# cvangysel/SERT

Hardware: AMD Instinct MI355X
Metric: training_pairs_per_sec (higher is better)
Workload: dtype f32; 1 GPU; C2 LSE: VectorSpaceLanguageModel (NCE z=10, Adam) V_w=100000 V_e=1000 d=128 window=10 batch=65536; global_batch=65536, per_gpu_batch=65536, parallelism=dp1, id_dtype=uint32, seed=0, instance_weights=1, dataset_instances=4194304, dataset_batches=64

## Files before the change

### include/sert_hip_debug.h

```cpp
#ifndef SERT_HIP_DEBUG_H
#define SERT_HIP_DEBUG_H

#include "sert_hip.h"

#ifdef __cplusplus
extern "C" {
#endif

int sert_debug_update_counts(sert_model* m, int64_t* out, int n);

int sert_debug_poison_scratch(sert_model* m);

int sert_debug_row_lists(const uint32_t* allbits, int world, int rank, int64_t num_batches, int64_t bit_words,
                         int64_t rows_per_rank, int64_t vocab, int64_t batch, int32_t* serve_cnt,
                         int32_t* fetch_cnt, int32_t* serve_rows, int32_t* fetch_rows, int32_t* union_rows,
                         int32_t* ptr, int32_t* ent, int64_t capacity, int64_t* sizes);

int sert_debug_word_index_sum(const void* ids, int id_bytes, int64_t num_batches, int B, int n, int vocab, int row_groups,
                              int dense_heavy, int64_t batch, const float* src, int d, float divisor, float* grad_out,
                              int64_t* stats);

int sert_debug_ll_rank_distributions(int device, const float* P, const int64_t* offsets, int64_t num_queries, int32_t V,
                                     int32_t k, int32_t* idx_out, float* score_out, float* joint_entropy_out,
                                     float* token_entropy_out, int32_t* status_out);

int sert_bench_gemm(int device, int ta, int tb, int epi, int M, int N, int K, int splits,
                    int iters, double* avg_us);

int sert_debug_gemm(int device, int ta, int tb, int epi, int M, int N, int K, const float* A, const float* B,
                    const float* bias, float* C);

int sert_debug_gemm_splitk(int device, int M, int N, int K, int splits, const float* A, const float* B, float* out);

int sert_debug_gemm_longk(int device, int tb, int M, int N, int K, int splits, const float* A, const float* B, float* C);

enum { SERT_MEMBENCH_COPY = 0, SERT_MEMBENCH_READ = 1, SERT_MEMBENCH_GATHER = 2, SERT_MEMBENCH_OPTIMIZER = 3 };
int sert_bench_memory(int device, int kind, size_t bytes, size_t table_bytes, int row_bytes,
                      int window, size_t gap_bytes, int blocks, int iters, double* avg_us);

struct sert_reval;
int sert_debug_reval_chunks(struct sert_reval* r);

// ... 5 lines not shown
```

### sert_amd/_capi.py

```python
import ctypes
import os

import numpy as np

_HERE = os.path.dirname(os.path.abspath(__file__))
LIB_PATH = os.environ.get('SERT_LIB') or os.path.join(_HERE, 'libsert_hip.so')

KIND_LOGLINEAR, KIND_VECTORSPACE, KIND_VECTORSPACE_SOFTMAX = 0, 1, 2
SPLIT_TRAIN, SPLIT_VALIDATE = 0, 1
LL_STATUS_DEVICE, LL_STATUS_HOST = 0, 1
REVAL_NDCG, REVAL_MAP, REVAL_RECIP_RANK, REVAL_P5, REVAL_NUM_REL_RET, REVAL_NUM_METRICS = 0, 1, 2, 3, 4, 5

T_RW, T_RE, T_W, T_B = 0, 1, 2, 3
T_STATE0_RW, T_STATE0_RE, T_STATE0_W, T_STATE0_B = 4, 5, 6, 7
T_STATE1_RW, T_STATE1_RE, T_STATE1_W, T_STATE1_B = 8, 9, 10, 11
T_GRAD_RW, T_GRAD_RE, T_GRAD_W, T_GRAD_B = 12, 13, 14, 15
T_ACT_H, T_ACT_T, T_ACT_DA, T_ACT_DH, T_ACT_ROWLOSS = 16, 17, 18, 19, 20

COMM_ID_BYTES = 128

EXPORTS = [
    'sert_create', 'sert_destroy', 'sert_last_error', 'sert_device_info', 'sert_device_count',
    'sert_set_tensor', 'sert_get_tensor', 'sert_tensor_size', 'sert_set_step', 'sert_get_step',
    'sert_set_eval_draws', 'sert_get_eval_draws', 'sert_negatives_of_step',
    'sert_upload_dataset', 'sert_train_batch', 'sert_hint_next_batch', 'sert_train_batches',
    'sert_eval_batch', 'sert_eval_batches',
    'sert_predict_project', 'sert_predict_tokens', 'sert_ll_rank_queries', 'sert_score_topk',
    'sert_reval_create', 'sert_reval_run', 'sert_reval_destroy',
    'sert_scorer_create', 'sert_scorer_destroy', 'sert_scorer_topk', 'sert_scorer_scores',
    'sert_host_alloc', 'sert_host_free',
    'sert_comm_unique_id', 'sert_comm_init', 'sert_comm_init_host', 'sert_comm_destroy', 'sert_comm_stats',
    'sert_synchronize', 'sert_timing_enable', 'sert_timing_reset', 'sert_timing_count',
    'sert_timing_name', 'sert_timing_avg_us', 'sert_timing_launches', 'sert_bench_gemm', 'sert_debug_gemm', 'sert_debug_gemm_splitk', 'sert_debug_gemm_longk', 'sert_bench_memory', 'sert_debug_row_lists', 'sert_debug_word_index_sum',
    'sert_debug_update_counts', 'sert_debug_poison_scratch', 'sert_debug_ll_rank_distributions', 'sert_debug_reval_chunks',
    'sert_profile_range_push', 'sert_profile_range_pop',
]


_F32P, _I64P = ctypes.POINTER(ctypes.c_float), ctypes.POINTER(ctypes.c_int64)
ALLTOALL_FN = ctypes.CFUNCTYPE(ctypes.c_int, ctypes.c_void_p, _F32P, _I64P, _I64P, _F32P, _I64P, _I64P)


class SertConfig(ctypes.Structure):
    _fields_ = [
        ('struct_size', ctypes.c_uint32),
        ('kind', ctypes.c_int32),
        ('batch_size', ctypes.c_int32),
        ('global_batch_size', ctypes.c_int32),
        ('window_size', ctypes.c_int32),
        ('vocab_size', ctypes.c_int32),
        ('num_entities', ctypes.c_int32),
        ('word_dim', ctypes.c_int32),
        ('entity_dim', ctypes.c_int32),
        ('num_negatives', ctypes.c_int32),
        ('id_bytes', ctypes.c_int32),
        ('device', ctypes.c_int32),
        ('keep_grads', ctypes.c_int32),
        ('deterministic', ctypes.c_int32),
        ('inference_only', ctypes.c_int32),
        ('lambda_', ctypes.c_float),
        ('lr', ctypes.c_float),
        ('beta1', ctypes.c_float),
        ('beta2', ctypes.c_float),
        ('eps', ctypes.c_float),
        ('seed', ctypes.c_uint64),
    ]

# ... 268 lines not shown
    def comm_stats(self):
        v = (ctypes.c_double * 8)()
        check(self._lib.sert_comm_stats(self._h, v, 8))
        return {'world': int(v[0]), 'exchange': {0: 'none', 1: 'zero1', 2: 'rows'}[int(v[1])],
                'bytes_per_step': float(v[2]), 'zero1_bytes_per_step': float(v[3]),
                'transport': {0: 'none', 1: 'rccl', 2: 'host'}[int(v[4])], 'steps': int(v[5]),
                'rows_fetched_per_batch': float(v[6]), 'rows_served_per_batch': float(v[7])}

    def synchronize(self):
        check(self._lib.sert_synchronize(self._h))

    def timing_enable(self, on=True):
        check(self._lib.sert_timing_enable(self._h, int(on)))

    def timing_launches(self):
        n = self._lib.sert_timing_count(self._h)
        return {self._lib.sert_timing_name(self._h, i).decode():
                self._lib.sert_timing_launches(self._h, i) for i in range(n)}

    def timing_reset(self):
        check(self._lib.sert_timing_reset(self._h))

    def poison_scratch(self):
        self._lib.sert_debug_poison_scratch.argtypes = [ctypes.c_void_p]
        check(self._lib.sert_debug_poison_scratch(self._h))

    def update_counts(self):
        v = (ctypes.c_int64 * 10)()
        self._lib.sert_debug_update_counts.argtypes = [ctypes.c_void_p, ctypes.POINTER(ctypes.c_int64), ctypes.c_int]
        check(self._lib.sert_debug_update_counts(self._h, v, 10))
        names = ('dense', 'lazy', 'skip_32_1', 'skip_64_1', 'skip_32_3', 'skip_64_2', 'skip_64_3', 'skip_64_4', 'skip_full', 'skip_sparse')
        return dict(zip(names, (int(x) for x in v)))

    def timings(self):
        n = self._lib.sert_timing_count(self._h)
        return {self._lib.sert_timing_name(self._h, i).decode():
                self._lib.sert_timing_avg_us(self._h, i) for i in range(n)}


def comm_unique_id():
    buf = ctypes.create_string_buffer(COMM_ID_BYTES)
    check(load().sert_comm_unique_id(buf))
    return buf.raw


def _concat_queries(token_lists):
    lengths = np.fromiter((len(t) for t in token_lists), dtype=np.int64, count=len(token_lists))
    offsets = np.zeros(len(token_lists) + 1, dtype=np.int64)
    np.cumsum(lengths, out=offsets[1:])
    tokens = np.ascontiguousarray(np.concatenate([np.asarray(t, dtype=np.int64) for t in token_lists])
                                  if len(token_lists) else np.zeros(0, np.int64), dtype=np.int32)
    return tokens, offsets


def _ll_rank_call(num_entities, offsets, k, call, num_tokens):
    q = offsets.size - 1
    kk = num_entities if k is None or k >= num_entities else int(k)
    idx = np.empty((q, kk), dtype=np.int32)
    score = np.empty((q, kk), dtype=np.float32)
    joint_h = np.empty(q, dtype=np.float32)
    token_h = np.empty(num_tokens, dtype=np.float32)
    status = np.empty(q, dtype=np.int32)
    outs = [a.ctypes.data for a in (idx, score, joint_h, token_h, status)]
    check(call(-1 if k is None else int(k), outs))
    return idx, score, joint_h, token_h, status, offsets

# ... 299 lines not shown
```

### sert_amd/csrc/host/api_data_train.inc

```

int sert_upload_dataset(sert_model* m, int split, const void* x, const int32_t* y_int,
                        const int64_t* csr_indptr, const int32_t* csr_indices,
                        const float* csr_data, const float* w, int64_t N) {
    if (!m) SERT_FAIL("null model");
    invalidate_speculation(m);
    m->hint_next = -1;
    if (split != SERT_SPLIT_TRAIN && split != SERT_SPLIT_VALIDATE) SERT_FAIL("bad split");
    if (N < 0) SERT_FAIL("negative instance count");
    if (N > 0 && !x) SERT_FAIL("x is null");
    if (N > 0 && !y_int && !(csr_indptr && csr_indices && csr_data)) SERT_FAIL("no labels given");
    if (is_vs(m) && N > 0 && !y_int) SERT_FAIL("vectorspace requires int labels (models.py:933-934)");
    SERT_HIP(hipSetDevice(m->cfg.device));
    if (N > 0) {
        const size_t toks = (size_t)N * m->cfg.window_size;
        const uint32_t Vw = (uint32_t)m->cfg.vocab_size;
        bool ok = true;
        SERT_ID_DISPATCH(m->cfg.id_bytes, {
            const IdT* xi = (const IdT*)x;
            uint32_t mx = 0;
            for (size_t i = 0; i < toks; ++i) mx = std::max<uint32_t>(mx, (uint32_t)xi[i]);
            ok = mx < Vw;
        });
        if (!ok) SERT_FAIL("token id >= vocab_size in x");
        const int32_t Ve = m->cfg.num_entities;
// ... 128 lines not shown
                d.dense_cnt_of.resize((size_t)nb);
                for (int64_t b = 0; b < nb; ++b) d.dense_cnt_of[(size_t)b] = wi.batches[(size_t)b].dense_cnt;
            }
            SERT_TRY(dmalloc(&d.idx_dense_words, hw.size()));
            SERT_HIP(hipMemcpyAsync(d.idx_dense_words, hw.data(), hw.size() * sizeof(int32_t), hipMemcpyHostToDevice, s));
            SERT_HIP(hipStreamSynchronize(s));
            if (!m->hpart)
                SERT_TRY(dmalloc(&m->hpart, (size_t)std::max(cdiv(B, heavy_rows_fused(B)), cdiv(B, kHeavyRowsPerBlock)) * kHeavyMax *
                                               (size_t)(is_vs(m) ? m->cfg.word_dim : m->cfg.num_entities)));
        } else {
            for (auto& bxx : wi.batches) bxx.dense_cnt = 0;
        }
        d.idx_batches = wi.batches;
        if ((size_t)wi.max_part_rows + 1 > m->wpart_rows) {
            (void)hipFree(m->wpart);
            m->wpart_rows = (size_t)wi.max_part_rows + 1;
            SERT_TRY(dmalloc(&m->wpart, m->wpart_rows * m->cfg.word_dim));
        }
    }
    SERT_HIP(hipStreamSynchronize(s));
    return 0;
}

int sert_train_batch(sert_model* m, int64_t batch_index, const int64_t* negatives, float* loss_out) {
    refresh_gemm_choice();
    if (!m) SERT_FAIL("null model");
    SERT_HIP(hipSetDevice(m->cfg.device));
    static const bool no_spin = variant_knob("SERT_NO_SPIN") != nullptr;
    const int64_t hint = m->hint_next;
    m->hint_next = -1;
    m->lazy_next = hint;
    auto prefetch_next = [&]() -> int {
        const DataSplit& ds = m->split[SERT_SPLIT_TRAIN];
        if (hint < 0 || m->timing.enabled || m->cfg.keep_grads) return 0;
        if ((hint + 1) * (int64_t)m->cfg.batch_size > ds.N) return 0;
        if (can_speculate_step(m)) {
            bool fused = false;
            SERT_TRY(step_forward_backward(m, ds, hint, nullptr, &fused));
            m->spec_fb_batch = hint;
            m->spec_fb_step = m->step;
        } else if (is_vs(m) && !is_fs(m)) {
            if (m->xr_on) SERT_TRY(xr_fetch_params(m, hint));
            SERT_TRY(vs_project(m, ds, hint));
            m->projected_batch = hint;
        } else if (m->xr_on) {
            SERT_TRY(xr_fetch_params(m, hint));
        }
        return 0;
    };
    if (m->timing.enabled || no_spin) {
        SERT_TRY(train_step_async(m, batch_index, negatives, m->d_loss));
        SERT_HIP(hipMemcpyAsync(m->h_loss, m->d_loss, 3 * sizeof(float), hipMemcpyDeviceToHost, m->stream));
        SERT_HIP(hipEventRecord(m->ev_loss, m->stream));
        SERT_TRY(prefetch_next());
        SERT_HIP(hipEventSynchronize(m->ev_loss));
        timing_collect(m);
        if (loss_out) *loss_out = m->h_loss[0];
        return 0;
    }
    SERT_TRY(train_step_async(m, batch_index, negatives, m->h_loss_dev, true));
    SERT_TRY(prefetch_next());
    const unsigned want = m->loss_seq;
    volatile unsigned* flag = reinterpret_cast<volatile unsigned*>(m->h_loss + 4);
    {
        const auto t_spin0 = std::chrono::steady_clock::now();
        double next_query_ms = 50.0;
        for (unsigned spins = 1; *flag != want; ++spins) {
            if ((spins & 0xfff) != 0) continue;
            const double waited_ms = std::chrono::duration<double, std::milli>(std::chrono::steady_clock::now() - t_spin0).count();
            if (waited_ms < next_query_ms) continue;
            next_query_ms = waited_ms + 50.0;
            const hipError_t q = hipStreamQuery(m->stream);
            if (q == hipSuccess) {
                if (*flag == want) break;
                SERT_FAIL("training step completed without publishing its loss");
            }
            if (q != hipErrorNotReady) SERT_HIP(q);
        }
    }
    __atomic_thread_fence(__ATOMIC_ACQUIRE);
    if (loss_out) *loss_out = m->h_loss[0];
    return 0;
}

int sert_hint_next_batch(sert_model* m, int64_t next_batch_index) {
    if (!m) SERT_FAIL("null model");
    m->hint_next = next_batch_index;
    return 0;
}

int sert_train_batches(sert_model* m, const int64_t* batch_indices, int64_t count, float* losses_out) {
    refresh_gemm_choice();
    if (!m || !batch_indices || count < 0) SERT_FAIL("bad argument");
    m->hint_next = -1;
// ... 191 lines not shown
```

### sert_amd/csrc/host/api_debug.inc

```

int sert_debug_poison_scratch(sert_model* m) {
    if (!m) SERT_FAIL("null argument");
    if (m->spec_fb_batch >= 0) SERT_FAIL("a run-ahead step is in flight (sert_hint_next_batch): its gradients live in the scratch");
    SERT_HIP(hipSetDevice(m->cfg.device));
    SERT_HIP(hipDeviceSynchronize());
    if (!m->gflat) return 0;
    std::vector<uint32_t> h(m->gflat_alloc, 0x7fc00000u);
    if (m->run_start) {
        const size_t V4 = round_up((size_t)m->cfg.num_entities, 4);
        for (size_t i = 0; i < V4; ++i) { h[m->gflat_count + i] = 0u; h[m->gflat_count + V4 + i] = 1u; }
    }
    SERT_HIP(hipMemcpy(m->gflat, h.data(), h.size() * sizeof(uint32_t), hipMemcpyHostToDevice));
    return 0;
}

int sert_debug_update_counts(sert_model* m, int64_t* out, int n) {
    if (!m || !out || n < 1 || n > 10) SERT_FAIL("bad argument");
    for (int i = 0; i < n; ++i) out[i] = m->upd_counts[i];
    return 0;
}

int sert_debug_row_lists(const uint32_t* allbits, int world, int rank, int64_t num_batches, int64_t bit_words,
                         int64_t rows_per_rank, int64_t vocab, int64_t batch, int32_t* serve_cnt, int32_t* fetch_cnt,
                         int32_t* serve_rows, int32_t* fetch_rows, int32_t* union_rows, int32_t* ptr, int32_t* ent,
                         int64_t capacity, int64_t* sizes) {
    if (!allbits || world < 1 || rank < 0 || rank >= world || batch < 0 || batch >= num_batches || !sizes)
        SERT_FAIL("bad argument");
    RowExchangeLists L;
    build_row_exchange(allbits, world, rank, num_batches, bit_words, rows_per_rank, vocab, L);
    const RowExchangeBatch& xb = L.batches[(size_t)batch];
    sizes[0] = xb.serve_total; sizes[1] = xb.fetch_total; sizes[2] = xb.nunion; sizes[3] = xb.nent; sizes[4] = L.max_xfer_rows;
    if (std::max<int64_t>(std::max(xb.serve_total, xb.fetch_total), std::max(xb.nunion + 1, xb.nent)) > capacity)
        SERT_FAIL("capacity too small");
    for (int q = 0; q < world; ++q) { serve_cnt[q] = xb.serve_cnt[(size_t)q]; fetch_cnt[q] = xb.fetch_cnt[(size_t)q]; }
    std::copy_n(L.serve_rows.begin() + xb.serve_off, xb.serve_total, serve_rows);
    std::copy_n(L.fetch_rows.begin() + xb.fetch_off, xb.fetch_total, fetch_rows);
    std::copy_n(L.union_rows.begin() + xb.union_off, xb.nunion, union_rows);
    std::copy_n(L.ptr.begin() + xb.ptr_off, xb.nunion + 1, ptr);
    std::copy_n(L.ent.begin() + xb.ent_off, xb.nent, ent);
    return 0;
}

int sert_debug_word_index_sum(const void* ids, int id_bytes, int64_t num_batches, int B, int n, int vocab, int row_groups,
                              int dense_heavy, int64_t batch, const float* src, int d, float divisor, float* grad_out,
                              int64_t* stats) {
    if (!ids || !src || !grad_out || !stats || num_batches <= 0 || B <= 0 || n <= 0 || vocab <= 0 || d <= 0 || batch < 0 ||
        batch >= num_batches || (id_bytes != 1 && id_bytes != 2 && id_bytes != 4))
        SERT_FAIL("bad argument");
    WordIndex wi;
    bool ok = true;
    SERT_ID_DISPATCH(id_bytes, ok = build_word_index<IdT>((const IdT*)ids, num_batches, B, n, vocab, false, wi,
// ... 353 lines not shown
```

### sert_amd/csrc/host/optimizer_and_loss.inc

```

static int reduce_rowloss(sert_model* m, hipStream_t st) {
    const int B = m->cfg.batch_size;
    int nb = std::min(kOptBlocks, cdiv(B, 256));
    m->loss_from_rows = false;
    if (is_vs(m) && !is_fs(m) && m->nce_loss_partials > 0) nb = m->nce_loss_partials;
    else if (!is_dp(m) && B <= 8192) {
        m->loss_from_rows = true;
        nb = B;
    } else hipLaunchKernelGGL(sum_partial, dim3(nb), dim3(256), 0, st, m->rowloss, (size_t)B, m->red_loss);
    if (is_dp(m))
        hipLaunchKernelGGL(partials_to_scalar, dim3(1), dim3(256), 0, st, m->red_loss, nb, m->g_loss);
    m->n_loss_partials = nb;
    return 0;
}

static void launch_stream_opt(sert_model* m, hipStream_t st, float* p, float* g, float* s0, float* s1, size_t count,
                              int nb, const AdamArgs& aa, const AdadeltaArgs& da, float* sq,
                              const uint32_t* bits, unsigned row_len, float* sq_new = nullptr) {
    const bool keep = m->cfg.keep_grads != 0;
    const int rows_mode = kRowsAll;
    if (is_vs(m)) {
        if (keep) hipLaunchKernelGGL((adam_l2<true>), dim3(nb), dim3(256), 0, st, p, g, s0, s1, count, aa, sq, bits, row_len, rows_mode, sq_new);
        else      hipLaunchKernelGGL((adam_l2<false>), dim3(nb), dim3(256), 0, st, p, g, s0, s1, count, aa, sq, bits, row_len, rows_mode, sq_new);
    } else {
// ... 261 lines not shown
        launch_stream_opt(m, ss, t.p, t.g, t.s0, t.s1, t.n, re_nb, aa, da, m->red_sq + re_sq_lo, nullptr, 1u,
                          m->re_sq + re_nxt * re_cap);
        m->re_sq_for[re_nxt] = m->step + 1;
        SERT_HIP(hipEventRecord(m->ev_re, ss));
        m->re_pending = true;
    }
    {
        ScopedTimer t(m, TG_FINALIZE);
        const float inv_batch = 1.0f / (float)c.global_batch_size;
        const float reg_scale = c.lambda_ > 0.f ? c.lambda_ / (2.0f * (float)c.global_batch_size) : 0.f;
        const float* lp = is_dp(m) ? m->g_loss : (m->loss_from_rows ? m->rowloss : m->red_loss);
        const int nl = is_dp(m) ? 1 : n_loss_partials;
        unsigned* flag = publish ? reinterpret_cast<unsigned*>(loss_dst + 4) : nullptr;
        if (tail_splits > 0) {
            if (m->dw_side_first) SERT_HIP(hipStreamWaitEvent(m->stream, m->ev_dense, 0));
            TailArgs ta;
            ta.part = m->part; ta.splits = tail_splits; ta.stride = m->tail_stride;
            ta.W = m->W; ta.b = m->b; ta.s0_w = m->s0_w; ta.s1_w = m->s1_w; ta.s0_b = m->s0_b; ta.s1_b = m->s1_b;
            ta.g_w = m->g_w; ta.g_b = m->g_b;
            ta.n_w = (unsigned)m->n_w; ta.n_b = (unsigned)m->n_b;
            ta.aa = aa;
            ta.loss_partials = lp; ta.n_loss = nl;
            ta.sq_partials = m->red_sq; ta.n_sq = n_sq;
            const bool alt = defer_re || (defer_small && re_nb > 0);
            ta.sq_alt = alt ? m->re_sq + re_cur * re_cap : nullptr;
            ta.sq_alt_lo = alt ? re_sq_lo : 0;
            ta.sq_alt_hi = alt ? re_sq_lo + re_nb : 0;
            ta.inv_batch = inv_batch; ta.reg_scale = reg_scale;
            ta.out = loss_dst; ta.host_flag = flag; ta.seq = publish ? ++m->loss_seq : 0u;
            ta.blk = m->tail_blk;
            if (++m->tail_launch_seq == 0) ++m->tail_launch_seq;
            ta.launch_seq = m->tail_launch_seq;
            const int nb = cdiv((int64_t)(m->n_w + m->n_b), 64);
            if (c.keep_grads) hipLaunchKernelGGL((vs_tail<true>), dim3(nb), dim3(1024), 0, m->stream, ta);
            else              hipLaunchKernelGGL((vs_tail<false>), dim3(nb), dim3(1024), 0, m->stream, ta);
        } else
        hipLaunchKernelGGL(finalize_loss, dim3(1), dim3(256), 0, m->stream, lp, nl, m->red_sq,
                           n_sq, inv_batch, reg_scale, loss_dst, flag, publish ? ++m->loss_seq : 0u,
                           is_dp(m) ? (const float*)m->g_sq : (const float*)nullptr);
    }
    if (any_ag) {
        SERT_HIP(hipEventRecord(m->ev_ag_done, m->comm_stream));
        SERT_HIP(hipStreamWaitEvent(m->stream, m->ev_ag_done, 0));
    }
    return 0;
}

static size_t zero_from(const sert_model* m) {
    static const bool all = variant_knob("SERT_ZERO_GRE") != nullptr;
    if (!all && m->cfg.kind == SERT_KIND_VECTORSPACE && !m->epart && m->n_re > 0 && m->g_re == m->gflat + m->ar_split)
        return m->ar_split + round_up(m->pt_pad[1], 4);
    return m->ar_split;
}

static bool egrad_writes_every_row(const sert_model* m) { return m->epart != nullptr || zero_from(m) > m->ar_split; }

static bool fused_prologue_applies_with(const sert_model* m, bool touched) {
    return is_vs(m) && !is_fs(m) && !m->timing.enabled && m->nstreams >= 2 && touched &&
           m->cfg.num_negatives > 0 && (m->gflat_alloc - zero_from(m)) % 4 == 0;
}
static bool fused_prologue_applies(const sert_model* m) { return fused_prologue_applies_with(m, m->use_touched); }
static void launch_fused_prologue(sert_model* m) {
    const int64_t count = (int64_t)m->cfg.batch_size * m->cfg.num_negatives;
    hipLaunchKernelGGL(vs_sample_negatives, dim3(grid_for((count + 3) / 4)), dim3(256), 0, m->stream, m->neg,
                       count, (int64_t)m->rank * count, (uint32_t)m->cfg.num_entities, m->cfg.seed,
                       (uint64_t)m->step * 2, reinterpret_cast<float4*>(m->gflat + zero_from(m)),
                       (m->gflat_alloc - zero_from(m)) / 4, (uint4*)nullptr, (size_t)0);
}
// ... 49 lines not shown
            SERT_HIP(hipMemsetAsync(m->gflat, 0, m->gflat_alloc * sizeof(float), pre));
        }
        if (!(is_vs(m) && !is_fs(m) && pre != m->stream)) SERT_TRY(owned_sum_of_squares(m, pre));
    }
    if (is_fs(m)) {
        SERT_TRY(fs_forward<true>(m, ds, batch_index));
        SERT_TRY(fs_backward(m, ds, batch_index));
        SERT_TRY(reduce_rowloss(m, m->stream));
    } else if (is_vs(m)) {
        if (!fused_pre) SERT_TRY(vs_negatives(m, negatives, (uint64_t)m->step * 2, pre));
        if (pre != m->stream) {
            SERT_HIP(hipEventRecord(m->ev_neg, pre));
            SERT_HIP(hipStreamWaitEvent(m->stream, m->ev_neg, 0));
            if (!have_neg && !fused_pre) SERT_TRY(owned_sum_of_squares(m, pre));
        }
        SERT_TRY(vs_loss<true>(m, ds, batch_index));
        SERT_TRY(vs_backward(m, ds, batch_index));
    } else {
        SERT_TRY(ll_forward<true>(m, ds, batch_index));
        SERT_TRY(ll_backward(m, ds, batch_index));
        SERT_TRY(reduce_rowloss(m, m->stream));
    }
    return 0;
}

static bool can_speculate_step(const sert_model* m) {
    if (m->timing.enabled || m->cfg.keep_grads) return false;
    if (is_dp(m)) {
        static const bool dp_off = variant_knob("SERT_DP_RUN_AHEAD") && atoi(variant_knob("SERT_DP_RUN_AHEAD")) == 0;
        return !dp_off && is_vs(m) && !is_fs(m);
    }
    if (is_vs(m) && !is_fs(m)) return use_touched_now(m) && fused_prologue_applies_with(m, true);
    return true;
}

static int train_step_async(sert_model* m, int64_t batch_index, const int64_t* negatives,
                            float* loss_dst, bool publish = false) {
    const DataSplit& ds = m->split[SERT_SPLIT_TRAIN];
    const int B = m->cfg.batch_size;
    if (m->cfg.inference_only) SERT_FAIL("model was created inference_only");
    if (m->comm_dead) SERT_FAIL("the communicator of this data-parallel model was destroyed");
    if (ds.N == 0) SERT_FAIL("no training data uploaded");
    if (batch_index < 0 || (batch_index + 1) * (int64_t)B > ds.N) SERT_FAIL("batch_index out of range");
    if (m->instep.on) ++m->instep.steps;
    const bool have_fb = negatives == nullptr && m->spec_fb_batch == batch_index && m->spec_fb_step == m->step &&
                         can_speculate_step(m);
    bool fused_pre = true;
    if (have_fb) m->spec_fb_batch = -1;
    else discard_run_ahead(m);
    const uint32_t* bits = ds.idx_touched_bits ? ds.idx_touched_bits + (size_t)batch_index * ds.bit_words : nullptr;
    if (!have_fb) SERT_TRY(step_forward_backward(m, ds, batch_index, negatives, &fused_pre));
    SERT_TRY(allreduce_rest(m));
    m->cur_touched_frac = (size_t)batch_index < ds.idx_batches.size()
                              ? (float)ds.idx_batches[(size_t)batch_index].num_distinct / (float)m->cfg.vocab_size : 1.f;
    const uint32_t* next_bits = nullptr;
    if (ds.idx_touched_bits && m->lazy_next >= 0 && (m->lazy_next + 1) * (int64_t)B <= ds.N)
        next_bits = ds.idx_touched_bits + (size_t)m->lazy_next * ds.bit_words;
    SERT_TRY(optimizer_and_loss(m, loss_dst, publish, bits, next_bits));
    if (is_dp(m)) m->comm_steps += 1;
    SERT_HIP(hipGetLastError());
    if (fused_pre) m->step_done_pending = true;
    else { SERT_HIP(hipEventRecord(m->ev_step_done, m->stream)); m->step_done_pending = false; }
    return 0;
}
```

### sert_amd/csrc/host/step_vectorspace.inc

```

static int reduce_rowloss(sert_model* m, hipStream_t st);

static int vs_negatives(sert_model* m, const int64_t* negatives, uint64_t stream_pos, hipStream_t st) {
    const auto& c = m->cfg;
    const int64_t count = (int64_t)c.batch_size * c.num_negatives;
    if (count == 0) return 0;
    if (negatives) {
        const int64_t Ve = c.num_entities;
        for (int64_t i = 0; i < count; ++i)
            if (negatives[i] < 0 || negatives[i] >= Ve) SERT_FAIL("negative sample out of range [0, num_entities)");
        SERT_HIP(hipMemcpyAsync(m->neg_stage, negatives, count * sizeof(int64_t),
                                hipMemcpyHostToDevice, st));
        hipLaunchKernelGGL(convert_i64_to_i32, dim3(grid_for(count)), dim3(256), 0, st,
                           m->neg_stage, m->neg, count);
    } else {
        const int64_t global_offset = (int64_t)m->rank * count;
        hipLaunchKernelGGL(vs_sample_negatives, dim3(grid_for((count + 3) / 4)), dim3(256), 0,
                           st, m->neg, count, global_offset, (uint32_t)c.num_entities,
                           c.seed, stream_pos);
    }
    return 0;
}

static int vs_project(sert_model* m, const DataSplit& ds, int64_t batch_index) {
    const auto& c = m->cfg;
    const int B = c.batch_size, n = c.window_size, dw = c.word_dim, de = c.entity_dim;
    const size_t row0 = (size_t)batch_index * B;
#ifdef SERT_VARIANTS
    if (m->proj_fused && gemm_x3_enabled() && vs_project_fused_ok(B, n, dw, de, m->n_rw)) {
        if (m->T_alt) std::swap(m->T, m->T_alt);
        ScopedTimer t(m, TG_GATHER);
        SERT_ID_DISPATCH(c.id_bytes, {
            const IdT* X = (const IdT*)ds.x + row0 * n;
            hipLaunchKernelGGL((vs_project_x3<IdT>), dim3(vs_project_grid(B, m->num_cus)), dim3(PJ_THREADS), 0, m->stream, X, (const float*)m->rw,
                               (const float*)m->W, (const float*)m->b, m->H, m->T, B, n, dw, de);
        });
        return 0;
    }
#endif
    {
        ScopedTimer t(m, TG_GATHER);
        SERT_ID_DISPATCH(c.id_bytes, {
            const IdT* X = (const IdT*)ds.x + row0 * n;
#ifdef SERT_VARIANTS
            const int nhot = (ds.idx_tok_slot && (size_t)batch_index < ds.dense_cnt_of.size()) ? ds.dense_cnt_of[(size_t)batch_index] : 0;
            if (dw % 4 == 0 && nhot > 0 && (size_t)nhot * dw * sizeof(float) <= 48 * 1024)
                hipLaunchKernelGGL((vs_gather_mean_hot<IdT>), dim3(std::min<int64_t>(grid_for((int64_t)B * dw / 4, 256, 1 << 20), 8 * m->num_cus)),
                                   dim3(256), (size_t)nhot * dw * sizeof(float), m->stream, X, (const uint8_t*)ds.idx_tok_slot + row0 * n,
                                   (const int32_t*)ds.idx_dense_words + (size_t)batch_index * kHeavyMax, nhot, (const float*)m->rw, m->H, B, n, dw);
            else
#endif
            if (dw % 4 == 0)
                hipLaunchKernelGGL((vs_gather_mean<IdT, 4>), dim3(grid_for((int64_t)B * dw / 4, 256, 1 << 20)),
                                   dim3(256), 0, m->stream, X, m->rw, m->H, B, n, dw);
            else
                hipLaunchKernelGGL((vs_gather_mean<IdT, 1>), dim3(grid_for((int64_t)B * dw, 256, 1 << 20)),
                                   dim3(256), 0, m->stream, X, m->rw, m->H, B, n, dw);
        });
    }
    if (m->T_alt) std::swap(m->T, m->T_alt);
    {
        ScopedTimer t(m, TG_GEMM_FWD);
#ifdef SERT_VARIANTS
        if (gemm_strip_ok(B, de, dw, dw, de, false, m->H, m->W))
            launch_gemm_strip<false, EPI_BIAS_TANH>(m->stream, m->H, m->W, m->T, m->b, B, de, dw, dw, de, de);
        else
#endif
            launch_gemm<false, false, EPI_BIAS_TANH>(m->stream, m->H, m->W, m->T, m->b, B, de, dw, dw,
                                                     de, de);
    }
    return 0;
}

static bool ext_events() {
    static const bool on = !(variant_knob("SERT_EXT_EVENTS") && atoi(variant_knob("SERT_EXT_EVENTS")) == 0);
    return on;
}

static bool side_heavy_mode(const sert_model* m);

static bool fork_late_mode(const sert_model* m) {
    static const bool on = !(variant_knob("SERT_FORK_LATE") && atoi(variant_knob("SERT_FORK_LATE")) == 0);
    return on && !side_heavy_mode(m) && ext_events() && !is_dp(m) && !m->timing.enabled && m->nstreams == 2 &&
           m->n_re <= ((size_t)1 << 22) && m->cfg.kind == SERT_KIND_VECTORSPACE;
}

static bool fork_at_nce(const sert_model* m) {
    static const bool on = variant_knob("SERT_FORK_AT") && !strncmp(variant_knob("SERT_FORK_AT"), "nce", 3);
    return on && fork_late_mode(m);
}
// ... 407 lines not shown
```

### sert_amd/csrc/kernels_opt.h

```cpp
#pragma once
#include "common.h"

namespace sert {

#ifndef SERT_OPT_BLOCKS
#define SERT_OPT_BLOCKS 2048
#endif
constexpr int kOptBlocks = SERT_OPT_BLOCKS;

struct AdamArgs {
    float l2k;
    float a_t;
    float b1, b2, eps;
};

__device__ __forceinline__ float sq_acc(float acc, float x) { return __builtin_fmaf(x, x, acc); }

__device__ __forceinline__ void adam_elem(float& p, float& g, float& m, float& v, const AdamArgs& a,
                                          float omb1, float omb2, float& ss, float& ss_new) {
#pragma clang fp contract(off)
    const float pv = p;
    const float l2 = a.l2k * pv;
    const float gv = g + l2;
    ss = sq_acc(ss, pv);
// ... 595 lines not shown
        b += __shfl_xor(b, off);
    }
    if ((threadIdx.x & 63) == 0) { red[0][threadIdx.x >> 6] = a; red[1][threadIdx.x >> 6] = b; }
    __syncthreads();
    const double loss_sum = (red[0][0] + red[0][1]) + (red[0][2] + red[0][3]);
    const double sq_sum = (red[1][0] + red[1][1]) + (red[1][2] + red[1][3]);
    if (threadIdx.x == 0) {
        const float data = (float)loss_sum * inv_batch;
        const float reg = reg_scale * (float)(sq_sum + (extra_sq ? (double)extra_sq[0] : 0.0));
        out[0] = data + reg;
        out[1] = data;
        out[2] = reg;
        if (host_flag) __hip_atomic_store(host_flag, seq, __ATOMIC_RELEASE, __HIP_MEMORY_SCOPE_SYSTEM);
    }
}

struct TailArgs {
    const float* part;
    int splits;
    unsigned long long stride;
    float *W, *b, *s0_w, *s1_w, *s0_b, *s1_b, *g_w, *g_b;
    unsigned n_w, n_b;
    AdamArgs aa;
    const float* loss_partials; int n_loss;
    const float* sq_partials; int n_sq;
    const float* sq_alt; int sq_alt_lo, sq_alt_hi;
    float inv_batch, reg_scale;
    float* out;
    unsigned* host_flag; unsigned seq;
    unsigned long long* blk;
    unsigned launch_seq;
};

template <bool STORE_G>
__global__ __launch_bounds__(1024) void vs_tail(const TailArgs t) {
    __shared__ float red[16][64];
    __shared__ double dred[2][16];
    const int l = threadIdx.x & 63, g = threadIdx.x >> 6;
    const unsigned count = t.n_w + t.n_b;
    const unsigned i = blockIdx.x * 64u + (unsigned)l;
    float a = 0.f;
    if (i < count) {
#pragma unroll 8
        for (int s = g; s < t.splits; s += 16) a += t.part[(size_t)s * t.stride + i];
    }
    red[g][l] = a;
    double ls = 0.0, sq = 0.0;
    for (int k = blockIdx.x * 1024 + threadIdx.x; k < t.n_loss; k += gridDim.x * 1024) ls += (double)t.loss_partials[k];
    for (int k = blockIdx.x * 1024 + threadIdx.x; k < t.n_sq; k += gridDim.x * 1024)
        sq += (double)((k >= t.sq_alt_lo && k < t.sq_alt_hi) ? t.sq_alt[k - t.sq_alt_lo] : t.sq_partials[k]);
    __syncthreads();
    if (g == 0 && i < count) {
        float q[4];
#pragma unroll
        for (int k = 0; k < 4; ++k) q[k] = (red[4 * k][l] + red[4 * k + 1][l]) + (red[4 * k + 2][l] + red[4 * k + 3][l]);
        float gg = ((q[0] + q[1]) + q[2]) + q[3];
        AdamArgs aa = t.aa;
        const float omb1 = 1.0f - aa.b1, omb2 = 1.0f - aa.b2;
        float ssf = 0.f;
        if (i < t.n_w) {
            float pp = t.W[i], m = t.s0_w[i], v = t.s1_w[i];
            { float unused = 0.f; adam_elem(pp, gg, m, v, aa, omb1, omb2, ssf, unused); }
            t.W[i] = pp; t.s0_w[i] = m; t.s1_w[i] = v;
            if (STORE_G) t.g_w[i] = gg;
            sq += (double)ssf;
        } else {
            const unsigned j = i - t.n_w;
            aa.l2k = 0.f;
            float pp = t.b[j], m = t.s0_b[j], v = t.s1_b[j];
            { float unused = 0.f; adam_elem(pp, gg, m, v, aa, omb1, omb2, ssf, unused); }
            t.b[j] = pp; t.s0_b[j] = m; t.s1_b[j] = v;
            if (STORE_G) t.g_b[j] = gg;
        }
    }
#pragma unroll
    for (int off = 32; off > 0; off >>= 1) {
        ls += __shfl_xor(ls, off);
        sq += __shfl_xor(sq, off);
    }
    if (l == 0) { dred[0][g] = ls; dred[1][g] = sq; }
    __syncthreads();
    if (threadIdx.x < 4) {
        const int which = threadIdx.x >> 1;
        double x = 0.0;
#pragma unroll
        for (int w = 0; w < 16; ++w) x += dred[which][w];
        const float hi = (float)x;
        const float piece = (threadIdx.x & 1) ? (float)(x - (double)hi) : hi;
        const unsigned long long word = ((unsigned long long)t.launch_seq << 32) | (unsigned long long)__float_as_uint(piece);
        __hip_atomic_store(t.blk + 4 * blockIdx.x + threadIdx.x, word, __ATOMIC_RELAXED, __HIP_MEMORY_SCOPE_AGENT);
    }
    if (blockIdx.x != gridDim.x - 1) return;
    __syncthreads();
    double c0 = 0.0, c1 = 0.0;
    for (unsigned k = threadIdx.x; k < gridDim.x; k += 1024) {
        unsigned long long w[4];
#pragma unroll
        for (int j = 0; j < 4; ++j)
            do { w[j] = __hip_atomic_load(t.blk + 4 * k + j, __ATOMIC_RELAXED, __HIP_MEMORY_SCOPE_AGENT); } while ((unsigned)(w[j] >> 32) != t.launch_seq);
        c0 += (double)__uint_as_float((unsigned)w[0]) + (double)__uint_as_float((unsigned)w[1]);
        c1 += (double)__uint_as_float((unsigned)w[2]) + (double)__uint_as_float((unsigned)w[3]);
    }
#pragma unroll
    for (int off = 32; off > 0; off >>= 1) {
        c0 += __shfl_xor(c0, off);
        c1 += __shfl_xor(c1, off);
    }
    if (l == 0) { dred[0][g] = c0; dred[1][g] = c1; }
    __syncthreads();
    if (threadIdx.x == 0) {
        double loss_sum = 0.0, sq_sum = 0.0;
#pragma unroll
        for (int w = 0; w < 16; ++w) { loss_sum += dred[0][w]; sq_sum += dred[1][w]; }
        const float data = (float)loss_sum * t.inv_batch;
        const float reg = t.reg_scale * (float)sq_sum;
        t.out[0] = data + reg;
        t.out[1] = data;
        t.out[2] = reg;
        if (t.host_flag) __hip_atomic_store(t.host_flag, t.seq, __ATOMIC_RELEASE, __HIP_MEMORY_SCOPE_SYSTEM);
    }
}

}
```

### sert_amd/csrc/kernels_vs.h

```cpp
#pragma once
#include "common.h"

namespace sert {

#ifndef SERT_GATHER_GC
#define SERT_GATHER_GC 10
#endif
template <typename IdT, int VEC>
__global__ __launch_bounds__(256) void vs_gather_mean(const IdT* __restrict__ X,
                                                      const float* __restrict__ Rw,
                                                      float* __restrict__ H, int B, int n, int d) {
    const int chunks = d / VEC;
    const int64_t total = (int64_t)B * chunks;
    const float fn = (float)n;
    for (int64_t tid = blockIdx.x * (int64_t)blockDim.x + threadIdx.x; tid < total;
         tid += (int64_t)gridDim.x * blockDim.x) {
        const int row = (int)(tid / chunks);
        const int c = (int)(tid - (int64_t)row * chunks) * VEC;
        const IdT* xr = X + (size_t)row * n;
        if (VEC == 4) {
            float4 a = make_float4(0.f, 0.f, 0.f, 0.f);
            constexpr int GC = SERT_GATHER_GC;
            for (int k0 = 0; k0 < n; k0 += GC) {
                size_t id[GC];
#pragma unroll
                for (int q = 0; q < GC; ++q) id[q] = (size_t)xr[min(k0 + q, n - 1)];
                float4 v[GC];
#pragma unroll
                for (int q = 0; q < GC; ++q) v[q] = *reinterpret_cast<const float4*>(Rw + id[q] * d + c);
#pragma unroll
                for (int q = 0; q < GC; ++q)
                    if (k0 + q < n) { a.x += v[q].x; a.y += v[q].y; a.z += v[q].z; a.w += v[q].w; }
            }
            a.x /= fn; a.y /= fn; a.z /= fn; a.w /= fn;
            *reinterpret_cast<float4*>(H + (size_t)row * d + c) = a;
        } else {
            float a = 0.f;
            for (int k = 0; k < n; ++k) a += Rw[(size_t)xr[k] * d + c];
            H[(size_t)row * d + c] = a / fn;
        }
    }
}

__device__ __forceinline__ void philox_round(uint32_t (&c)[4], uint32_t k0, uint32_t k1) {
    const uint64_t p0 = (uint64_t)0xD2511F53u * c[0];
    const uint64_t p1 = (uint64_t)0xCD9E8D57u * c[2];
    const uint32_t n0 = (uint32_t)(p1 >> 32) ^ c[1] ^ k0;
    const uint32_t n1 = (uint32_t)p1;
    const uint32_t n2 = (uint32_t)(p0 >> 32) ^ c[3] ^ k1;
    const uint32_t n3 = (uint32_t)p0;
    c[0] = n0; c[1] = n1; c[2] = n2; c[3] = n3;
}
__device__ __forceinline__ void philox4x32_10(uint32_t (&c)[4], uint32_t k0, uint32_t k1) {
#pragma unroll
    for (int r = 0; r < 10; ++r) {
        philox_round(c, k0, k1);
        k0 += 0x9E3779B9u;
        k1 += 0xBB67AE85u;
    }
}
__global__ __launch_bounds__(256) void vs_build_cand(const int32_t* __restrict__ y, const int32_t* __restrict__ neg, int B, int z,
                                                     int32_t* __restrict__ cand) {
    const int c1 = z + 1, total = B * c1;
    for (int i = blockIdx.x * 256 + threadIdx.x; i < total; i += gridDim.x * 256) {
        const int row = i / c1, j = i - row * c1;
        cand[i] = j ? neg[(size_t)row * z + (j - 1)] : y[row];
    }
}

__global__ void vs_sample_negatives(int32_t* __restrict__ neg, int64_t count, int64_t global_offset,
                                    uint32_t num_entities, uint64_t seed, uint64_t step,
                                    float4* __restrict__ zero_f = nullptr, size_t nzf4 = 0,
                                    uint4* __restrict__ zero_b = nullptr, size_t nzb16 = 0) {
    {
// ... 398 lines not shown
```

### sert_amd/csrc/model.h

```cpp
#pragma once
#include <vector>
#include <string>
#include "common.h"
#include "word_index.h"
#include "kernels_xchg.h"
#include "../../include/sert_hip.h"
#include "../../include/sert_hip_debug.h"

namespace sert {

struct DataSplit {
    int64_t N = 0;
    void* x = nullptr;
    int32_t* y = nullptr;
    int64_t* csr_indptr = nullptr;
    int32_t* csr_indices = nullptr;
    float* csr_data = nullptr;
    int64_t nnz = 0;
    int64_t max_labels_per_row = 0;
    float* w = nullptr;
    float* labfix = nullptr;
    int32_t* idx_rows = nullptr;
    int4* idx_items = nullptr;
    int4* idx_heavy = nullptr;
    int32_t* idx_bundles = nullptr;
    int32_t* idx_uwords = nullptr;
    int32_t* idx_slots = nullptr;
    int32_t* idx_rows_div = nullptr;
    uint32_t* idx_touched_bits = nullptr;
    uint4* idx_dense_counts = nullptr;
    int32_t* idx_dense_words = nullptr;
    uint8_t* idx_tok_slot = nullptr;
    std::vector<int32_t> dense_cnt_of;
    int64_t bit_words = 0;
    std::vector<BatchIndex> idx_batches;
};

enum TimingGroup {
// ... 121 lines not shown
    int32_t *eg_entries = nullptr, *eg_offs = nullptr;
    int eg_sub_rows = 0, eg_num_sub = 0, eg_subs_per_group = 0, eg_groups = 0, eg_ranges = 0, eg_er_shift = 0;
    int32_t *sort_hist = nullptr, *sort_bin_total = nullptr;
    int32_t *sort_k_tmp = nullptr, *sort_v_tmp = nullptr;
    int sort_bits = 1;
    float *G = nullptr;
    float *Z = nullptr;
    float *J = nullptr;
    float *DG = nullptr;

    float* wpart = nullptr;
    float* hpart = nullptr;
    size_t wpart_rows = 0;
    float* part = nullptr;
    size_t part_count = 0;
    float2* ll_tokstat = nullptr; float* ll_lse = nullptr; float2* ll_jstat = nullptr;
    float4* ll_rowinfo = nullptr; float* ll_rpart = nullptr; float* ll_r = nullptr;
    bool use_touched = false;

    float* Zu = nullptr;
    float* dZu = nullptr;
    size_t zu_rows = 0;
    float* zpart = nullptr;
    size_t zpart_rows = 0;
    bool ll_dedup = false;
    float* ll_rsum = nullptr;
    int ll_U = 0;
    float* skbuf = nullptr;
    size_t skbuf_count = 0;
    unsigned long long* tail_blk = nullptr;
    unsigned tail_launch_seq = 0;
    int tail_splits = 0;
    size_t tail_stride = 0;
    float* red_loss = nullptr;
    float* red_sq = nullptr;
    float* d_loss = nullptr;
    float* h_loss = nullptr;
    float* d_losses = nullptr;
    int64_t d_losses_cap = 0;

    float *pred_a = nullptr, *pred_b = nullptr;
    void* pred_ids = nullptr;
    size_t pred_a_cap = 0, pred_b_cap = 0, pred_ids_cap = 0;

    sert::DataSplit split[2];

    int64_t step = 0;
    int64_t eval_draws = 0;

    size_t pt_pad[4] = {0, 0, 0, 0};
    size_t pt_sc[4] = {0, 0, 0, 0};
    bool pt_big[4] = {false, false, false, false};
    bool pt_sharded[4] = {false, false, false, false};
    size_t ar_split = 0;
    size_t rest_off = 0;
    float* g_sq = nullptr;
    float* sq_scratch = nullptr;

    int rank = 0, world = 1;
    void* comm = nullptr;
    bool comm_dead = false;
    sert_alltoall_fn host_ar = nullptr;
    void* host_ar_user = nullptr;
    float *host_send = nullptr, *host_recv = nullptr;
    size_t host_send_cap = 0, host_recv_cap = 0;

// ... 52 lines not shown
```

Before: 293.7 million pairs/s.

## Fold deferred optimizer tail into next batch's gather-mean kernel launch

The vs_tail kernel (split reduction, Adam update on the dense part, loss finalize) is no longer launched on its own when the next batch will be speculated. Its launch is deferred and merged into the next vs_gather_mean launch: the first blocks of the combined grid run the tail body with 256-thread workgroups and the remaining blocks do the gather. This saves one kernel launch per step and lets the tail and the gather overlap on the GPU. In exchange the tail runs with smaller workgroups, each thread handling several splits, and the code gains deferral state that must be flushed on every other path. The tail reads W/b parameters while the gather reads rw, so correctness relies on those being disjoint.

Result: faster. 304.6 million pairs/s (median of 6 runs) (+3.7%).

```diff
diff --git a/include/sert_hip_debug.h b/include/sert_hip_debug.h
--- a/include/sert_hip_debug.h
+++ b/include/sert_hip_debug.h
@@ -8,6 +8,8 @@
 #endif
 
 int sert_debug_update_counts(sert_model* m, int64_t* out, int n);
+
+int sert_debug_tail_counts(sert_model* m, int64_t* out, int n);
 
 int sert_debug_poison_scratch(sert_model* m);
 
diff --git a/sert_amd/_capi.py b/sert_amd/_capi.py
--- a/sert_amd/_capi.py
+++ b/sert_amd/_capi.py
@@ -32,7 +32,7 @@
     'sert_comm_unique_id', 'sert_comm_init', 'sert_comm_init_host', 'sert_comm_destroy', 'sert_comm_stats',
     'sert_synchronize', 'sert_timing_enable', 'sert_timing_reset', 'sert_timing_count',
     'sert_timing_name', 'sert_timing_avg_us', 'sert_timing_launches', 'sert_bench_gemm', 'sert_debug_gemm', 'sert_debug_gemm_splitk', 'sert_debug_gemm_longk', 'sert_bench_memory', 'sert_debug_row_lists', 'sert_debug_word_index_sum',
-    'sert_debug_update_counts', 'sert_debug_poison_scratch', 'sert_debug_ll_rank_distributions', 'sert_debug_reval_chunks',
+    'sert_debug_update_counts', 'sert_debug_tail_counts', 'sert_debug_poison_scratch', 'sert_debug_ll_rank_distributions', 'sert_debug_reval_chunks',
     'sert_profile_range_push', 'sert_profile_range_pop',
 ]
 
@@ -367,6 +367,12 @@
         names = ('dense', 'lazy', 'skip_32_1', 'skip_64_1', 'skip_32_3', 'skip_64_2', 'skip_64_3', 'skip_64_4', 'skip_full', 'skip_sparse')
         return dict(zip(names, (int(x) for x in v)))
 
+    def tail_counts(self):
+        v = (ctypes.c_int64 * 2)()
+        self._lib.sert_debug_tail_counts.argtypes = [ctypes.c_void_p, ctypes.POINTER(ctypes.c_int64), ctypes.c_int]
+        check(self._lib.sert_debug_tail_counts(self._h, v, 2))
+        return {'alone': int(v[0]), 'in_gather': int(v[1])}
+
     def timings(self):
         n = self._lib.sert_timing_count(self._h)
         return {self._lib.sert_timing_name(self._h, i).decode():
diff --git a/sert_amd/csrc/host/api_data_train.inc b/sert_amd/csrc/host/api_data_train.inc
--- a/sert_amd/csrc/host/api_data_train.inc
+++ b/sert_amd/csrc/host/api_data_train.inc
@@ -184,14 +184,16 @@
     m->lazy_next = hint;
     auto prefetch_next = [&]() -> int {
         const DataSplit& ds = m->split[SERT_SPLIT_TRAIN];
-        if (hint < 0 || m->timing.enabled || m->cfg.keep_grads) return 0;
-        if ((hint + 1) * (int64_t)m->cfg.batch_size > ds.N) return 0;
-        if (can_speculate_step(m)) {
+        if (will_run_ahead(m, hint)) {
             bool fused = false;
             SERT_TRY(step_forward_backward(m, ds, hint, nullptr, &fused));
             m->spec_fb_batch = hint;
             m->spec_fb_step = m->step;
-        } else if (is_vs(m) && !is_fs(m)) {
+            return 0;
+        }
+        if (hint < 0 || m->timing.enabled || m->cfg.keep_grads) return 0;
+        if ((hint + 1) * (int64_t)m->cfg.batch_size > ds.N) return 0;
+        if (is_vs(m) && !is_fs(m)) {
             if (m->xr_on) SERT_TRY(xr_fetch_params(m, hint));
             SERT_TRY(vs_project(m, ds, hint));
             m->projected_batch = hint;
@@ -210,8 +212,13 @@
         if (loss_out) *loss_out = m->h_loss[0];
         return 0;
     }
-    SERT_TRY(train_step_async(m, batch_index, negatives, m->h_loss_dev, true));
-    SERT_TRY(prefetch_next());
+    static const bool no_fold = variant_knob("SERT_TAIL_IN_GATHER") && atoi(variant_knob("SERT_TAIL_IN_GATHER")) == 0;
+    m->tail_defer = !no_fold && !is_dp(m) && is_vs(m) && !is_fs(m) && will_run_ahead(m, hint);
+    int rc = train_step_async(m, batch_index, negatives, m->h_loss_dev, true);
+    m->tail_defer = false;
+    if (rc == 0) rc = prefetch_next();
+    flush_pending_tail(m);
+    if (rc != 0) return rc;
     const unsigned want = m->loss_seq;
     volatile unsigned* flag = reinterpret_cast<volatile unsigned*>(m->h_loss + 4);
     {
diff --git a/sert_amd/csrc/host/api_debug.inc b/sert_amd/csrc/host/api_debug.inc
--- a/sert_amd/csrc/host/api_debug.inc
+++ b/sert_amd/csrc/host/api_debug.inc
@@ -17,6 +17,12 @@
 int sert_debug_update_counts(sert_model* m, int64_t* out, int n) {
     if (!m || !out || n < 1 || n > 10) SERT_FAIL("bad argument");
     for (int i = 0; i < n; ++i) out[i] = m->upd_counts[i];
+    return 0;
+}
+
+int sert_debug_tail_counts(sert_model* m, int64_t* out, int n) {
+    if (!m || !out || n < 1 || n > 2) SERT_FAIL("bad argument");
+    for (int i = 0; i < n; ++i) out[i] = m->tail_counts[i];
     return 0;
 }
 
diff --git a/sert_amd/csrc/host/optimizer_and_loss.inc b/sert_amd/csrc/host/optimizer_and_loss.inc
--- a/sert_amd/csrc/host/optimizer_and_loss.inc
+++ b/sert_amd/csrc/host/optimizer_and_loss.inc
@@ -317,8 +317,15 @@
             if (++m->tail_launch_seq == 0) ++m->tail_launch_seq;
             ta.launch_seq = m->tail_launch_seq;
             const int nb = cdiv((int64_t)(m->n_w + m->n_b), 64);
-            if (c.keep_grads) hipLaunchKernelGGL((vs_tail<true>), dim3(nb), dim3(1024), 0, m->stream, ta);
-            else              hipLaunchKernelGGL((vs_tail<false>), dim3(nb), dim3(1024), 0, m->stream, ta);
+            if (m->tail_defer && publish && !c.keep_grads) {
+                m->tail_args = ta;
+                m->tail_nb = nb;
+                m->tail_pending = true;
+            } else {
+                ++m->tail_counts[0];
+                if (c.keep_grads) hipLaunchKernelGGL((vs_tail<true>), dim3(nb), dim3(1024), 0, m->stream, ta);
+                else              hipLaunchKernelGGL((vs_tail<false>), dim3(nb), dim3(1024), 0, m->stream, ta);
+            }
         } else
         hipLaunchKernelGGL(finalize_loss, dim3(1), dim3(256), 0, m->stream, lp, nl, m->red_sq,
                            n_sq, inv_batch, reg_scale, loss_dst, flag, publish ? ++m->loss_seq : 0u,
@@ -434,6 +441,10 @@
     }
     if (is_vs(m) && !is_fs(m)) return use_touched_now(m) && fused_prologue_applies_with(m, true);
     return true;
+}
+
+static bool will_run_ahead(const sert_model* m, int64_t hint) {
+    return hint >= 0 && (hint + 1) * (int64_t)m->cfg.batch_size <= m->split[SERT_SPLIT_TRAIN].N && can_speculate_step(m);
 }
 
 static int train_step_async(sert_model* m, int64_t batch_index, const int64_t* negatives,
diff --git a/sert_amd/csrc/host/step_vectorspace.inc b/sert_amd/csrc/host/step_vectorspace.inc
--- a/sert_amd/csrc/host/step_vectorspace.inc
+++ b/sert_amd/csrc/host/step_vectorspace.inc
@@ -22,12 +22,21 @@
     return 0;
 }
 
+static void flush_pending_tail(sert_model* m) {
+    if (!m->tail_pending) return;
+    m->tail_pending = false;
+    ScopedTimer t(m, TG_FINALIZE);
+    ++m->tail_counts[0];
+    hipLaunchKernelGGL((vs_tail<false>), dim3(m->tail_nb), dim3(1024), 0, m->stream, m->tail_args);
+}
+
 static int vs_project(sert_model* m, const DataSplit& ds, int64_t batch_index) {
     const auto& c = m->cfg;
     const int B = c.batch_size, n = c.window_size, dw = c.word_dim, de = c.entity_dim;
     const size_t row0 = (size_t)batch_index * B;
 #ifdef SERT_VARIANTS
     if (m->proj_fused && gemm_x3_enabled() && vs_project_fused_ok(B, n, dw, de, m->n_rw)) {
+        flush_pending_tail(m);
         if (m->T_alt) std::swap(m->T, m->T_alt);
         ScopedTimer t(m, TG_GATHER);
         SERT_ID_DISPATCH(c.id_bytes, {
@@ -44,18 +53,26 @@
             const IdT* X = (const IdT*)ds.x + row0 * n;
 #ifdef SERT_VARIANTS
             const int nhot = (ds.idx_tok_slot && (size_t)batch_index < ds.dense_cnt_of.size()) ? ds.dense_cnt_of[(size_t)batch_index] : 0;
-            if (dw % 4 == 0 && nhot > 0 && (size_t)nhot * dw * sizeof(float) <= 48 * 1024)
+            if (dw % 4 == 0 && nhot > 0 && (size_t)nhot * dw * sizeof(float) <= 48 * 1024) {
+                flush_pending_tail(m);
                 hipLaunchKernelGGL((vs_gather_mean_hot<IdT>), dim3(std::min<int64_t>(grid_for((int64_t)B * dw / 4, 256, 1 << 20), 8 * m->num_cus)),
                                    dim3(256), (size_t)nhot * dw * sizeof(float), m->stream, X, (const uint8_t*)ds.idx_tok_slot + row0 * n,
                                    (const int32_t*)ds.idx_dense_words + (size_t)batch_index * kHeavyMax, nhot, (const float*)m->rw, m->H, B, n, dw);
-            else
-#endif
-            if (dw % 4 == 0)
+            } else
+#endif
+            if (dw % 4 == 0 && m->tail_pending) {
+                m->tail_pending = false;
+                ++m->tail_counts[1];
+                hipLaunchKernelGGL((vs_gather_mean_tail<IdT>), dim3(m->tail_nb + grid_for((int64_t)B * dw / 4, 256, 1 << 20)),
+                                   dim3(256), 0, m->stream, X, m->rw, m->H, B, n, dw, m->tail_args, (unsigned)m->tail_nb);
+            } else if (dw % 4 == 0) {
                 hipLaunchKernelGGL((vs_gather_mean<IdT, 4>), dim3(grid_for((int64_t)B * dw / 4, 256, 1 << 20)),
                                    dim3(256), 0, m->stream, X, m->rw, m->H, B, n, dw);
-            else
+            } else {
+                flush_pending_tail(m);
                 hipLaunchKernelGGL((vs_gather_mean<IdT, 1>), dim3(grid_for((int64_t)B * dw, 256, 1 << 20)),
                                    dim3(256), 0, m->stream, X, m->rw, m->H, B, n, dw);
+            }
         });
     }
     if (m->T_alt) std::swap(m->T, m->T_alt);
diff --git a/sert_amd/csrc/kernels_opt.h b/sert_amd/csrc/kernels_opt.h
--- a/sert_amd/csrc/kernels_opt.h
+++ b/sert_amd/csrc/kernels_opt.h
@@ -651,25 +651,42 @@
     unsigned launch_seq;
 };
 
-template <bool STORE_G>
-__global__ __launch_bounds__(1024) void vs_tail(const TailArgs t) {
-    __shared__ float red[16][64];
-    __shared__ double dred[2][16];
-    const int l = threadIdx.x & 63, g = threadIdx.x >> 6;
+template <bool STORE_G, int NT>
+__device__ __forceinline__ void vs_tail_body(const TailArgs& t, const unsigned blk, const unsigned nblk, float (*red)[64],
+                                             double (*dred)[16]) {
+    static_assert(NT == 1024 || NT == 256, "vs_tail's and vs_gather_mean_tail's workgroups");
+    constexpr int J = 1024 / NT, NW = NT / 64;
+    const int l = threadIdx.x & 63, w = threadIdx.x >> 6;
     const unsigned count = t.n_w + t.n_b;
-    const unsigned i = blockIdx.x * 64u + (unsigned)l;
-    float a = 0.f;
+    const unsigned i = blk * 64u + (unsigned)l;
+    float a[J];
+#pragma unroll
+    for (int j = 0; j < J; ++j) a[j] = 0.f;
     if (i < count) {
-#pragma unroll 8
-        for (int s = g; s < t.splits; s += 16) a += t.part[(size_t)s * t.stride + i];
-    }
-    red[g][l] = a;
-    double ls = 0.0, sq = 0.0;
-    for (int k = blockIdx.x * 1024 + threadIdx.x; k < t.n_loss; k += gridDim.x * 1024) ls += (double)t.loss_partials[k];
-    for (int k = blockIdx.x * 1024 + threadIdx.x; k < t.n_sq; k += gridDim.x * 1024)
-        sq += (double)((k >= t.sq_alt_lo && k < t.sq_alt_hi) ? t.sq_alt[k - t.sq_alt_lo] : t.sq_partials[k]);
+        int s0 = 0;
+        constexpr int kTrips = J == 1 ? 8 : 4;
+#pragma unroll kTrips
+        for (; s0 + 16 <= t.splits; s0 += 16) {
+#pragma unroll
+            for (int j = 0; j < J; ++j) a[j] += t.part[(size_t)(s0 + w + NW * j) * t.stride + i];
+        }
+#pragma unroll
+        for (int j = 0; j < J; ++j)
+            if (s0 + w + NW * j < t.splits) a[j] += t.part[(size_t)(s0 + w + NW * j) * t.stride + i];
+    }
+#pragma unroll
+    for (int j = 0; j < J; ++j) red[w + NW * j][l] = a[j];
+    double ls[J], sq[J];
+#pragma unroll
+    for (int j = 0; j < J; ++j) {
+        const int vt = (int)threadIdx.x + NT * j;
+        ls[j] = 0.0; sq[j] = 0.0;
+        for (int k = blk * 1024 + vt; k < t.n_loss; k += nblk * 1024) ls[j] += (double)t.loss_partials[k];
+        for (int k = blk * 1024 + vt; k < t.n_sq; k += nblk * 1024)
+            sq[j] += (double)((k >= t.sq_alt_lo && k < t.sq_alt_hi) ? t.sq_alt[k - t.sq_alt_lo] : t.sq_partials[k]);
+    }
     __syncthreads();
-    if (g == 0 && i < count) {
+    if (w == 0 && i < count) {
         float q[4];
 #pragma unroll
         for (int k = 0; k < 4; ++k) q[k] = (red[4 * k][l] + red[4 * k + 1][l]) + (red[4 * k + 2][l] + red[4 * k + 3][l]);
@@ -682,7 +699,7 @@
             { float unused = 0.f; adam_elem(pp, gg, m, v, aa, omb1, omb2, ssf, unused); }
             t.W[i] = pp; t.s0_w[i] = m; t.s1_w[i] = v;
             if (STORE_G) t.g_w[i] = gg;
-            sq += (double)ssf;
+            sq[0] += (double)ssf;
         } else {
             const unsigned j = i - t.n_w;
             aa.l2k = 0.f;
@@ -693,44 +710,51 @@
         }
     }
 #pragma unroll
-    for (int off = 32; off > 0; off >>= 1) {
-        ls += __shfl_xor(ls, off);
-        sq += __shfl_xor(sq, off);
-    }
-    if (l == 0) { dred[0][g] = ls; dred[1][g] = sq; }
+    for (int j = 0; j < J; ++j) {
+#pragma unroll
+        for (int off = 32; off > 0; off >>= 1) {
+            ls[j] += __shfl_xor(ls[j], off);
+            sq[j] += __shfl_xor(sq[j], off);
+        }
+        if (l == 0) { dred[0][w + NW * j] = ls[j]; dred[1][w + NW * j] = sq[j]; }
+    }
     __syncthreads();
     if (threadIdx.x < 4) {
         const int which = threadIdx.x >> 1;
         double x = 0.0;
 #pragma unroll
-        for (int w = 0; w < 16; ++w) x += dred[which][w];
+        for (int k = 0; k < 16; ++k) x += dred[which][k];
         const float hi = (float)x;
         const float piece = (threadIdx.x & 1) ? (float)(x - (double)hi) : hi;
         const unsigned long long word = ((unsigned long long)t.launch_seq << 32) | (unsigned long long)__float_as_uint(piece);
-        __hip_atomic_store(t.blk + 4 * blockIdx.x + threadIdx.x, word, __ATOMIC_RELAXED, __HIP_MEMORY_SCOPE_AGENT);
-    }
-    if (blockIdx.x != gridDim.x - 1) return;
+        __hip_atomic_store(t.blk + 4 * blk + threadIdx.x, word, __ATOMIC_RELAXED, __HIP_MEMORY_SCOPE_AGENT);
+    }
+    if (blk != nblk - 1) return;
     __syncthreads();
-    double c0 = 0.0, c1 = 0.0;
-    for (unsigned k = threadIdx.x; k < gridDim.x; k += 1024) {
-        unsigned long long w[4];
-#pragma unroll
-        for (int j = 0; j < 4; ++j)
-            do { w[j] = __hip_atomic_load(t.blk + 4 * k + j, __ATOMIC_RELAXED, __HIP_MEMORY_SCOPE_AGENT); } while ((unsigned)(w[j] >> 32) != t.launch_seq);
-        c0 += (double)__uint_as_float((unsigned)w[0]) + (double)__uint_as_float((unsigned)w[1]);
-        c1 += (double)__uint_as_float((unsigned)w[2]) + (double)__uint_as_float((unsigned)w[3]);
-    }
-#pragma unroll
-    for (int off = 32; off > 0; off >>= 1) {
-        c0 += __shfl_xor(c0, off);
-        c1 += __shfl_xor(c1, off);
-    }
-    if (l == 0) { dred[0][g] = c0; dred[1][g] = c1; }
+    double c0[J], c1[J];
+#pragma unroll
+    for (int j = 0; j < J; ++j) {
+        c0[j] = 0.0; c1[j] = 0.0;
+        for (unsigned k = threadIdx.x + NT * j; k < nblk; k += 1024) {
+            unsigned long long wd[4];
+#pragma unroll
+            for (int q = 0; q < 4; ++q)
+                do { wd[q] = __hip_atomic_load(t.blk + 4 * k + q, __ATOMIC_RELAXED, __HIP_MEMORY_SCOPE_AGENT); } while ((unsigned)(wd[q] >> 32) != t.launch_seq);
+            c0[j] += (double)__uint_as_float((unsigned)wd[0]) + (double)__uint_as_float((unsigned)wd[1]);
+            c1[j] += (double)__uint_as_float((unsigned)wd[2]) + (double)__uint_as_float((unsigned)wd[3]);
+        }
+#pragma unroll
+        for (int off = 32; off > 0; off >>= 1) {
+            c0[j] += __shfl_xor(c0[j], off);
+            c1[j] += __shfl_xor(c1[j], off);
+        }
+        if (l == 0) { dred[0][w + NW * j] = c0[j]; dred[1][w + NW * j] = c1[j]; }
+    }
     __syncthreads();
     if (threadIdx.x == 0) {
         double loss_sum = 0.0, sq_sum = 0.0;
 #pragma unroll
-        for (int w = 0; w < 16; ++w) { loss_sum += dred[0][w]; sq_sum += dred[1][w]; }
+        for (int k = 0; k < 16; ++k) { loss_sum += dred[0][k]; sq_sum += dred[1][k]; }
         const float data = (float)loss_sum * t.inv_batch;
         const float reg = t.reg_scale * (float)sq_sum;
         t.out[0] = data + reg;
@@ -740,4 +764,11 @@
     }
 }
 
-}
+template <bool STORE_G>
+__global__ __launch_bounds__(1024) void vs_tail(const TailArgs t) {
+    __shared__ float red[16][64];
+    __shared__ double dred[2][16];
+    vs_tail_body<STORE_G, 1024>(t, blockIdx.x, gridDim.x, red, dred);
+}
+
+}
diff --git a/sert_amd/csrc/kernels_vs.h b/sert_amd/csrc/kernels_vs.h
--- a/sert_amd/csrc/kernels_vs.h
+++ b/sert_amd/csrc/kernels_vs.h
@@ -1,5 +1,6 @@
 #pragma once
 #include "common.h"
+#include "kernels_opt.h"
 
 namespace sert {
 
@@ -7,14 +8,13 @@
 #define SERT_GATHER_GC 10
 #endif
 template <typename IdT, int VEC>
-__global__ __launch_bounds__(256) void vs_gather_mean(const IdT* __restrict__ X,
-                                                      const float* __restrict__ Rw,
-                                                      float* __restrict__ H, int B, int n, int d) {
+__device__ __forceinline__ void vs_gather_mean_body(const IdT* __restrict__ X, const float* __restrict__ Rw,
+                                                    float* __restrict__ H, int B, int n, int d, unsigned blk, unsigned nblk) {
     const int chunks = d / VEC;
     const int64_t total = (int64_t)B * chunks;
     const float fn = (float)n;
-    for (int64_t tid = blockIdx.x * (int64_t)blockDim.x + threadIdx.x; tid < total;
-         tid += (int64_t)gridDim.x * blockDim.x) {
+    for (int64_t tid = blk * (int64_t)blockDim.x + threadIdx.x; tid < total;
+         tid += (int64_t)nblk * blockDim.x) {
         const int row = (int)(tid / chunks);
         const int c = (int)(tid - (int64_t)row * chunks) * VEC;
         const IdT* xr = X + (size_t)row * n;
@@ -40,6 +40,25 @@
             H[(size_t)row * d + c] = a / fn;
         }
     }
+}
+template <typename IdT, int VEC>
+__global__ __launch_bounds__(256) void vs_gather_mean(const IdT* __restrict__ X,
+                                                      const float* __restrict__ Rw,
+                                                      float* __restrict__ H, int B, int n, int d) {
+    vs_gather_mean_body<IdT, VEC>(X, Rw, H, B, n, d, blockIdx.x, gridDim.x);
+}
+
+template <typename IdT>
+__global__ __launch_bounds__(256) void vs_gather_mean_tail(const IdT* __restrict__ X, const float* __restrict__ Rw,
+                                                           float* __restrict__ H, int B, int n, int d, const TailArgs t,
+                                                           unsigned tail_blocks) {
+    __shared__ float red[16][64];
+    __shared__ double dred[2][16];
+    if (blockIdx.x < tail_blocks) {
+        vs_tail_body<false, 256>(t, blockIdx.x, tail_blocks, red, dred);
+        return;
+    }
+    vs_gather_mean_body<IdT, 4>(X, Rw, H, B, n, d, blockIdx.x - tail_blocks, gridDim.x - tail_blocks);
 }
 
 __device__ __forceinline__ void philox_round(uint32_t (&c)[4], uint32_t k0, uint32_t k1) {
diff --git a/sert_amd/csrc/model.h b/sert_amd/csrc/model.h
--- a/sert_amd/csrc/model.h
+++ b/sert_amd/csrc/model.h
@@ -4,6 +4,7 @@
 #include "common.h"
 #include "word_index.h"
 #include "kernels_xchg.h"
+#include "kernels_opt.h"
 #include "../../include/sert_hip.h"
 #include "../../include/sert_hip_debug.h"
 
@@ -191,6 +192,11 @@
     unsigned tail_launch_seq = 0;
     int tail_splits = 0;
     size_t tail_stride = 0;
+    bool tail_defer = false;
+    bool tail_pending = false;
+    sert::TailArgs tail_args;
+    int tail_nb = 0;
+    int64_t tail_counts[2] = {0, 0};
     float* red_loss = nullptr;
     float* red_sq = nullptr;
     float* d_loss = nullptr;
```
